# bao1029p/celestia-app

Measured on AMD Instinct MI355X. Metric: EDS+DAH squares/sec (128→256 sq, node) + RS GB/s & NMT SHA-256 hashes/sec, higher is better.
Workload: dtype u8; 1 GPU; 128x128 ODS -> 256x256 EDS + NMT row/col roots + DAH (configs[1]); k=128, global_batch=256, parallelism=squares sharded over 1 GPU(s), no collective, ods_layout=in place (Q0 of the EDS buffer)

## Files before the change

celestia-app_amd/csrc/dagpu.cpp:

```cpp
#include <hip/hip_runtime.h>
#include <stdint.h>
#include <stdio.h>
#include <stdlib.h>
#include <string.h>

#include <algorithm>
#include <cmath>
#include <map>
#include <mutex>
#include <string>
#include <vector>

#include "../../include/dagpu.h"
#include "host_sha256.hpp"
#include "kernels.hpp"
#include "runtime.hpp"

using namespace dagpu;

namespace {

size_t eds_bytes(uint64_t k) { return 4ull * k * k * kSS; }
size_t ods_bytes(uint64_t k) { return 1ull * k * k * kSS; }

int enqueue_rs(dagpu_ctx* ctx, uint32_t k, size_t n, const uint8_t* d_ods, uint8_t* d_eds,
               hipStream_t s, hipEvent_t ev_rows = nullptr) {
  const long w = 2L * k;
  const long esq = (long)eds_bytes(k);
  EncodeArgs ra{};
  if (d_ods) {
    ra.in = d_ods;
    ra.in_sq_stride = (long)ods_bytes(k);
    ra.in_vec_stride = (long)k * kSS;
    ra.in_shard_stride = kSS;
    ra.copy = d_eds;
    ra.copy_sq_stride = esq;
    ra.copy_vec_stride = w * kSS;
    ra.copy_shard_stride = kSS;
  } else {
    ra.in = d_eds;
    ra.in_sq_stride = esq;
    ra.in_vec_stride = w * kSS;
    ra.in_shard_stride = kSS;
    ra.copy = nullptr;
  }
  ra.out = d_eds + (long)k * kSS;
  ra.out_sq_stride = esq;
  ra.out_vec_stride = w * kSS;
  ra.out_shard_stride = kSS;
  ra.nsq = (long)n;
  ra.nvec = k;
  ra.nchunk = 1;
  ra.shard_bytes = kSS;
  {
    ProfScope p(ctx, 0, s);
    HIP_TRY(ctx, launch_rs_encode((int)k, ra, s));
  }
  stage_mark(ctx, DAGPU_STAGE_ROWS, s);
  if (ev_rows) HIP_TRY(ctx, hipEventRecord(ev_rows, s));
  EncodeArgs ca{};
  ca.in = d_eds;
  ca.in_sq_stride = esq;
  ca.in_vec_stride = kSS;
  ca.in_shard_stride = w * kSS;
  ca.out = d_eds + (long)k * w * kSS;
  ca.out_sq_stride = esq;
  ca.out_vec_stride = kSS;
  ca.out_shard_stride = w * kSS;
  ca.copy = nullptr;
  ca.nsq = (long)n;
  ca.nvec = w;
  ca.nchunk = 1;
  ca.shard_bytes = kSS;
  {
    ProfScope p(ctx, 1, s);
    HIP_TRY(ctx, launch_rs_encode((int)k, ca, s));
  }
  stage_mark(ctx, DAGPU_STAGE_COLS, s);
  return DAGPU_OK;
}

int enqueue_roots(dagpu_ctx* ctx, uint32_t k, size_t n, const uint8_t* d_eds, uint8_t* d_rr,
                  uint8_t* d_cr, uint8_t* d_dah, int32_t* d_status, void* d_ws, hipStream_t s) {
  SquareArgs sa{};
  sa.eds = d_eds;
  sa.eds_sq_stride = (long)eds_bytes(k);
  sa.k = (int)k;
  sa.nsq = (long)n;
  nmt_workspace_carve(sa, d_ws);
  sa.row_roots = d_rr;
  sa.col_roots = d_cr;
  sa.dah = d_dah;
  sa.status = d_status;
  sa.k = (int)k;
  sa.nsq = (long)n;
  HIP_TRY(ctx, hipMemsetAsync(d_status, 0, n * sizeof(int32_t), s));
  {
    ProfScope p(ctx, 2, s);
    HIP_TRY(ctx, launch_nmt_leaves(sa, s));
  }
  stage_mark(ctx, DAGPU_STAGE_LEAVES, s);
  {
    ProfScope p(ctx, 3, s);
    HIP_TRY(ctx, launch_nmt_trees(sa, s));
  }
  stage_mark(ctx, DAGPU_STAGE_TREES, s);
  if (d_dah) {
    ProfScope p(ctx, 4, s);
    HIP_TRY(ctx, launch_dah(sa, s));
  }
  stage_mark(ctx, DAGPU_STAGE_DAH, s);
  return DAGPU_OK;
}

size_t pipeline_chunk(uint32_t k, size_t n) {
  size_t m = (size_t(128) << 20) / ods_bytes(k);
  const long v = sw_long(SW_PIPELINE_CHUNK);
  if (v > 0) m = (size_t)v;
  return m < 1 ? 1 : (m > n ? n : m);
}

int finish_status(dagpu_ctx* ctx, const int32_t* st, size_t n, int32_t* status) {
  int first = DAGPU_OK;
  for (size_t i = 0; i < n; i++) {
    int v = (st[i] & kStatusPushOrder) ? DAGPU_ERR_PUSH_ORDER : DAGPU_OK;
    if (status) status[i] = v;
    if (v && !first) first = v;
  }
  if (first) set_err(ctx, first, "invalid push order: namespaces of original data square are not sorted");
  return first;
}

int run_group_pipelined(dagpu_ctx* ctx, uint32_t k, size_t n, size_t m, const uint8_t* ods,
                        uint8_t* eds_out, uint8_t* rr, uint8_t* cr, uint8_t* dah, int32_t* status) {
  const size_t w = 2 * (size_t)k;
  const size_t rb = w * kNodeSize, ob = ods_bytes(k), eb = eds_bytes(k);
  const size_t wsb = dagpu_workspace_size(k, m);
  hipStream_t s = ctx->stream, cs = ctx->copy_stream;
  HIP_TRY(ctx, ctx->ods.ensure(2 * m * ob));
  HIP_TRY(ctx, ctx->eds.ensure(2 * m * eb));
  HIP_TRY(ctx, ctx->rr.ensure(2 * m * rb));
  HIP_TRY(ctx, ctx->cr.ensure(2 * m * rb));
  HIP_TRY(ctx, ctx->dah.ensure(2 * m * 32));
  HIP_TRY(ctx, ctx->status.ensure(2 * m * sizeof(int32_t)));
  HIP_TRY(ctx, ctx->ws.ensure(2 * wsb));
  const size_t hslot = m * (2 * rb + 32 + sizeof(int32_t));
  HIP_TRY(ctx, ctx->h_out.ensure(2 * hslot));
  std::vector<int32_t> st(n);
  const size_t nchunks = (n + m - 1) / m;
  auto slot_dev = [&](DevBuf& b, size_t per, int slot) { return (uint8_t*)b.p + slot * m * per; };
  auto slot_host = [&](int slot) { return (uint8_t*)ctx->h_out.p + slot * hslot; };
  auto drain = [&](size_t c) -> int {
    const int slot = (int)(c & 1);
    const size_t off = c * m, cnt = (n - off < m) ? n - off : m;
    HIP_TRY(ctx, hipEventSynchronize(ctx->ev_done[slot]));
    const uint8_t* h = slot_host(slot);
    memcpy(rr + off * rb, h, cnt * rb);
    memcpy(cr + off * rb, h + m * rb, cnt * rb);
    memcpy(dah + off * 32, h + 2 * m * rb, cnt * 32);
    memcpy(st.data() + off, h + 2 * m * rb + m * 32, cnt * sizeof(int32_t));
    return DAGPU_OK;
  };
  for (size_t c = 0; c < nchunks; c++) {
    const int slot = (int)(c & 1);
    const size_t off = c * m, cnt = (n - off < m) ? n - off : m;
    if (c >= 2) {
      int rc = drain(c - 2);
      if (rc) return rc;
      HIP_TRY(ctx, hipStreamWaitEvent(cs, ctx->ev_done[slot], 0));
    }
    uint8_t* d_ods = slot_dev(ctx->ods, ob, slot);
    uint8_t* d_eds = slot_dev(ctx->eds, eb, slot);
    uint8_t* d_rr = slot_dev(ctx->rr, rb, slot);
    uint8_t* d_cr = slot_dev(ctx->cr, rb, slot);
    uint8_t* d_dah = slot_dev(ctx->dah, 32, slot);
    int32_t* d_st = (int32_t*)slot_dev(ctx->status, sizeof(int32_t), slot);
    HIP_TRY(ctx, hipMemcpyAsync(d_ods, ods + off * ob, cnt * ob, hipMemcpyHostToDevice, cs));
    HIP_TRY(ctx, hipEventRecord(ctx->ev_loaded[slot], cs));
    HIP_TRY(ctx, hipStreamWaitEvent(s, ctx->ev_loaded[slot], 0));
    int rc = enqueue_rs(ctx, k, cnt, d_ods, d_eds, s);
    if (rc) return rc;
    rc = enqueue_roots(ctx, k, cnt, d_eds, d_rr, d_cr, d_dah, d_st, (uint8_t*)ctx->ws.p + slot * wsb, s);
    if (rc) return rc;
    if (eds_out)
      HIP_TRY(ctx, hipMemcpyAsync(eds_out + off * eb, d_eds, cnt * eb, hipMemcpyDeviceToHost, s));
    uint8_t* h = slot_host(slot);
    HIP_TRY(ctx, hipMemcpyAsync(h, d_rr, cnt * rb, hipMemcpyDeviceToHost, s));
    HIP_TRY(ctx, hipMemcpyAsync(h + m * rb, d_cr, cnt * rb, hipMemcpyDeviceToHost, s));
    HIP_TRY(ctx, hipMemcpyAsync(h + 2 * m * rb, d_dah, cnt * 32, hipMemcpyDeviceToHost, s));
    HIP_TRY(ctx, hipMemcpyAsync(h + 2 * m * rb + m * 32, d_st, cnt * sizeof(int32_t), hipMemcpyDeviceToHost, s));
    HIP_TRY(ctx, hipEventRecord(ctx->ev_done[slot], s));
  }
  for (size_t c = nchunks >= 2 ? nchunks - 2 : 0; c < nchunks; c++) {
    int rc = drain(c);
// ... 275 lines not shown
                            row_roots + o_root[i], col_roots + o_root[i], dah + 32 * i, st.data());
    if (rc && rc != DAGPU_ERR_PUSH_ORDER) return rc;
    for (size_t t = i; t < j; t++) {
      if (status) status[t] = st[t - i];
      if (st[t - i] && !first) first = st[t - i];
    }
    i = j;
  }
  return first;
}

int dagpu_extend_rs_device(dagpu_ctx* ctx, uint32_t k, size_t n, const uint8_t* d_ods,
                           uint8_t* d_eds, void* stream) {
  if (!ctx || !d_eds) return DAGPU_ERR_ARG;
  int rc = check_k(ctx, k);
  if (rc) return rc;
  return enqueue_rs(ctx, k, n, d_ods, d_eds, (hipStream_t)stream);
}

int dagpu_roots_device(dagpu_ctx* ctx, uint32_t k, size_t n, const uint8_t* d_eds,
                       uint8_t* d_row_roots, uint8_t* d_col_roots, uint8_t* d_dah,
                       int32_t* d_status, void* d_workspace, void* stream) {
  if (!ctx || !d_eds || !d_row_roots || !d_col_roots || !d_dah || !d_status || !d_workspace)
    return DAGPU_ERR_ARG;
  int rc = check_k(ctx, k);
  if (rc) return rc;
  return enqueue_roots(ctx, k, n, d_eds, d_row_roots, d_col_roots, d_dah, d_status, d_workspace,
                       (hipStream_t)stream);
}

extern "C++" {
namespace dagpu {

namespace {
const char* const kSwNames[SW_COUNT] = {
    "DAGPU_PIPELINE_CHUNK", "DAGPU_PIPE_SLICES", "DAGPU_REPAIR_FILL", "DAGPU_SPLIT_SQUARE", "DAGPU_SPLIT_OVERLAP",
    "DAGPU_DAH_SPLIT",      "DAGPU_DEC_SLICED",  "DAGPU_ENC_SLICED",  "DAGPU_ENC_SLICED2",  "DAGPU_GF16_WIDE"};
thread_local const SwSnapshot* tl_sw = nullptr;
}

const char* sw(Switch s) {
  if (s < 0 || s >= SW_COUNT) return nullptr;
  if (tl_sw) return tl_sw->set[s] ? tl_sw->v[s] : nullptr;
  return getenv(kSwNames[s]);
}

long sw_long(Switch s, long dflt) {
  const char* e = sw(s);
  return e ? atol(e) : dflt;
}

void sw_snapshot(SwSnapshot* out) {
  for (int i = 0; i < SW_COUNT; i++) {
    const char* e = getenv(kSwNames[i]);
    out->set[i] = e != nullptr;
    out->v[i][0] = 0;
    if (e) snprintf(out->v[i], sizeof out->v[i], "%s", e);
  }
}

void sw_bind(const SwSnapshot* snap) { tl_sw = snap; }

hipEvent_t ev_take(dagpu_ctx* c) {
  std::lock_guard<std::mutex> g(c->ev_mu);
  if (!c->ev_pool.empty()) {
    hipEvent_t e = c->ev_pool.back();
    c->ev_pool.pop_back();
    return e;
  }
  hipEvent_t e = nullptr;
  if (hipEventCreateWithFlags(&e, hipEventDisableTiming) != hipSuccess) return nullptr;
  return e;
}

void ev_give(dagpu_ctx* c, hipEvent_t e) {
  if (!e) return;
  std::lock_guard<std::mutex> g(c->ev_mu);
  c->ev_pool.push_back(e);
}

size_t pipe_slices(dagpu_ctx* ctx, uint32_t k, size_t n) {
  const long env = sw_long(SW_PIPE_SLICES);
  if (ctx->prof) return 1;
  size_t s = env > 0 ? (size_t)env : (k >= 128 && n >= 64 ? 4 : 1);
  while (s > 1 && n / s < 8) s >>= 1;
  return s < 1 ? 1 : s;
}

hipStream_t side_stream(dagpu_ctx* ctx, hipStream_t s, int which) {
  std::lock_guard<std::mutex> g(ctx->side_mu);
  dagpu_ctx::Side* sd = nullptr;
  for (auto& p : ctx->side)
    if (p.caller == s) sd = &p;
  if (!sd) {
    if (ctx->side.size() >= dagpu_ctx::kMaxSideStreams) {
      const size_t i = (size_t)((((uint64_t)(uintptr_t)s) * 0x9E3779B97F4A7C15ull) >> 32) % ctx->side.size();
      sd = &ctx->side[i];
    } else {
      ctx->side.emplace_back();
      sd = &ctx->side.back();
      sd->caller = s;
    }
  }
  hipStream_t* slot = which == 1 ? &sd->rs_hi : &sd->rs;
  if (!*slot) {
    hipError_t e;
    if (which == 1) {
      int lo = 0, hi = 0;
      (void)hipDeviceGetStreamPriorityRange(&lo, &hi);
      e = hipStreamCreateWithPriority(slot, hipStreamNonBlocking, hi);
    } else {
      e = hipStreamCreateWithFlags(slot, hipStreamNonBlocking);
    }
    if (e != hipSuccess) {
      *slot = nullptr;
      return nullptr;
    }
  }
  return *slot;
}

}
}

int dagpu_extend_batch_device(dagpu_ctx* ctx, uint32_t k, size_t n, const uint8_t* d_ods,
                              uint8_t* d_eds, uint8_t* d_row_roots, uint8_t* d_col_roots,
                              uint8_t* d_dah, int32_t* d_status, void* d_workspace,
                              void* stream) {
  if (!ctx || !d_eds || !d_row_roots || !d_col_roots || !d_dah || !d_status || !d_workspace)
    return DAGPU_ERR_ARG;
  int rc = check_k(ctx, k);
  if (rc) return rc;
  const size_t S = pipe_slices(ctx, k, n);
  hipStream_t s = (hipStream_t)stream;
  if (S <= 1) {
    rc = enqueue_rs(ctx, k, n, d_ods, d_eds, s);
    if (rc) return rc;
    return enqueue_roots(ctx, k, n, d_eds, d_row_roots, d_col_roots, d_dah, d_status, d_workspace, s);
  }
  std::vector<hipEvent_t> ev(S + 1, nullptr);
  for (auto& e : ev)
    if (!(e = ev_take(ctx))) {
      for (auto x : ev) ev_give(ctx, x);
      return set_err(ctx, DAGPU_ERR_DEVICE, "hipEventCreate failed");
    }
  auto done = [&](int r) {
    for (auto x : ev) ev_give(ctx, x);
    return r;
  };
  hipStream_t rs = side_stream(ctx, s, 0);
  if (!rs) return done(set_err(ctx, DAGPU_ERR_DEVICE, "hipStreamCreate failed"));
  const size_t w = 2 * (size_t)k;
  if (hipEventRecord(ev[S], s) != hipSuccess || hipStreamWaitEvent(rs, ev[S], 0) != hipSuccess)
    return done(set_err(ctx, DAGPU_ERR_DEVICE, "pipeline fork failed"));
  std::vector<size_t> cut(S + 1);
  for (size_t i = 0; i <= S; i++) cut[i] = n * i / S;
  for (size_t i = 0; i < S; i++) {
    const size_t a = cut[i], b = cut[i + 1];
    rc = enqueue_rs(ctx, k, b - a, d_ods ? d_ods + a * ods_bytes(k) : nullptr, d_eds + a * eds_bytes(k), rs);
    if (rc) return done(rc);
    if (hipEventRecord(ev[i], rs) != hipSuccess) return done(set_err(ctx, DAGPU_ERR_DEVICE, "hipEventRecord failed"));
  }
  for (size_t i = 0; i < S; i++) {
    const size_t a = cut[i], b = cut[i + 1];
    if (hipStreamWaitEvent(s, ev[i], 0) != hipSuccess)
      return done(set_err(ctx, DAGPU_ERR_DEVICE, "hipStreamWaitEvent failed"));
    rc = enqueue_roots(ctx, k, b - a, d_eds + a * eds_bytes(k), d_row_roots + a * w * kNodeSize,
                       d_col_roots + a * w * kNodeSize, d_dah + a * 32, d_status + a, (uint8_t*)d_workspace, s);
    if (rc) return done(rc);
  }
  return done(DAGPU_OK);
}

int dagpu_roots(dagpu_ctx* ctx, uint32_t k, const uint8_t* eds, uint8_t* row_roots,
                uint8_t* col_roots, uint8_t* dah) {
  if (!ctx || !eds || !row_roots || !col_roots || !dah) return DAGPU_ERR_ARG;
  std::lock_guard<std::mutex> g(ctx->mu);
  (void)hipSetDevice(ctx->device);
  int rc = check_k(ctx, k);
  if (rc) return rc;
  hipStream_t s = ctx->stream;
  HostResults res;
  HIP_TRY(ctx, ctx->eds.ensure(eds_bytes(k)));
  HIP_TRY(ctx, res.alloc(ctx, k, 1));
  HIP_TRY(ctx, ctx->ws.ensure(dagpu_workspace_size(k, 1)));
  HIP_TRY(ctx, hipMemcpyAsync(ctx->eds.p, eds, eds_bytes(k), hipMemcpyHostToDevice, s));
  rc = enqueue_roots(ctx, k, 1, (const uint8_t*)ctx->eds.p, res.rr, res.cr, res.dah, res.st, ctx->ws.p, s);
  if (rc) return rc;
  HIP_TRY(ctx, res.download(ctx, s));
  HIP_TRY(ctx, hipStreamSynchronize(s));
  int32_t st = 0;
  res.deliver(ctx, row_roots, col_roots, dah, &st);
  if (st & kStatusPushOrder)
    return set_err(ctx, DAGPU_ERR_PUSH_ORDER, "invalid push order: namespaces of original data square are not sorted");
  return DAGPU_OK;
}

int dagpu_encode(dagpu_ctx* ctx, uint32_t k, size_t nvec, size_t shard_size,
                 const uint8_t* data, uint8_t* parity) {
  if (!ctx || (nvec && (!data || !parity))) return DAGPU_ERR_ARG;
  if (shard_size == 0 || shard_size % 64)
    return set_err(ctx, DAGPU_ERR_SHARE_SIZE, "shard size must be a multiple of 64");
  std::lock_guard<std::mutex> g(ctx->mu);
  (void)hipSetDevice(ctx->device);
  int rc = check_codec_k(ctx, k);
  if (rc) return rc;
  if (nvec == 0) return DAGPU_OK;
  const size_t bytes = (size_t)k * shard_size * nvec;
  hipStream_t s = ctx->stream;
  HIP_TRY(ctx, ctx->ods.ensure(bytes));
  HIP_TRY(ctx, ctx->eds.ensure(bytes));
  HIP_TRY(ctx, hipMemcpyAsync(ctx->ods.p, data, bytes, hipMemcpyHostToDevice, s));
  EncodeArgs ea{};
  ea.in = (const uint8_t*)ctx->ods.p;
  ea.out = (uint8_t*)ctx->eds.p;
  ea.copy = nullptr;
  ea.in_sq_stride = 0;
  ea.out_sq_stride = 0;
  ea.in_vec_stride = (long)k * (long)shard_size;
  ea.out_vec_stride = (long)k * (long)shard_size;
  ea.in_shard_stride = (long)shard_size;
  ea.out_shard_stride = (long)shard_size;
  ea.nsq = 1;
  ea.nvec = (long)nvec;
  ea.nchunk = (long)((shard_size + 511) / 512);
  ea.shard_bytes = (long)shard_size;
  HIP_TRY(ctx, launch_rs_encode((int)k, ea, s));
  HIP_TRY(ctx, hipMemcpyAsync(parity, ctx->eds.p, bytes, hipMemcpyDeviceToHost, s));
  HIP_TRY(ctx, hipStreamSynchronize(s));
  return DAGPU_OK;
}

int dagpu_decode(dagpu_ctx* ctx, uint32_t k, size_t nvec, size_t shard_size, uint8_t* shards,
                 const uint8_t* present) {
  if (!ctx || (nvec && (!shards || !present))) return DAGPU_ERR_ARG;
  if (shard_size == 0 || shard_size % 64)
    return set_err(ctx, DAGPU_ERR_SHARE_SIZE, "shard size must be a multiple of 64");
  std::lock_guard<std::mutex> g(ctx->mu);
  (void)hipSetDevice(ctx->device);
  int rc = check_codec_k(ctx, k);
  if (rc) return rc;
  if (nvec == 0) return DAGPU_OK;
  const size_t n = 2 * (size_t)k;
  const size_t bytes = n * shard_size * nvec;
  hipStream_t s = ctx->stream;
  HIP_TRY(ctx, ctx->eds.ensure(bytes));
  HIP_TRY(ctx, ctx->ods.ensure(n * nvec));
  const size_t errb = (size_t)rs_err_bytes((int)k) * nvec;
  HIP_TRY(ctx, ctx->ws.ensure(errb + 3 * nvec * sizeof(int32_t) + 256));
  HIP_TRY(ctx, ctx->status.ensure(sizeof(int32_t)));
  HIP_TRY(ctx, hipMemcpyAsync(ctx->eds.p, shards, bytes, hipMemcpyHostToDevice, s));
  HIP_TRY(ctx, hipMemcpyAsync(ctx->ods.p, present, n * nvec, hipMemcpyHostToDevice, s));
  HIP_TRY(ctx, hipMemsetAsync(ctx->status.p, 0, sizeof(int32_t), s));
  DecodeArgs da{};
// ... 821 lines not shown
```

celestia-app_amd/csrc/kernels.hpp:

```cpp
#pragma once
#include <hip/hip_runtime.h>
#include <stdint.h>

#include "switches.hpp"

namespace dagpu {

constexpr int kShareSize = 512;
constexpr int kNsSize = 29;
constexpr int kNodeSize = 90;
constexpr int kDigest = 32;
constexpr int kMaxK = 8192;
constexpr int kMaxCodecK = 32768;
constexpr int kMaxSplitK = 2 * kMaxK;
constexpr int kMinWideSplitParts = 8;

constexpr long rs_err_tab_off(int k) { return 4L * k; }
constexpr long rs_err_elem_bytes(int k) { return k <= 1024 ? 80 : 32; }
constexpr long rs_err_bytes(int k) { return k <= 128 ? 256 : 4L * k + 2L * k * rs_err_elem_bytes(k); }

constexpr int kStatusPushOrder = 1;

struct EncodeArgs {
  const uint8_t* in;
// ... 95 lines not shown
hipError_t launch_leo8_decode_only(const DecodeArgs& a, hipStream_t s, bool mark_present);
bool leo8_decode_sliced_applicable(const DecodeArgs& a);
hipError_t launch_leo8_decode128_sliced(const DecodeArgs& a, hipStream_t s);

hipError_t launch_leo16_encode(int k, const EncodeArgs& a, hipStream_t s);
hipError_t launch_leo16_errlocs(const DecodeArgs& a, hipStream_t s);
hipError_t launch_leo16_decode_only(const DecodeArgs& a, hipStream_t s, bool mark_present);
hipError_t launch_leo16w_encode(int k, const EncodeArgs& a, hipStream_t s);
hipError_t launch_leo16w_errlocs(const DecodeArgs& a, hipStream_t s);
hipError_t launch_leo16w_decode_only(const DecodeArgs& a, hipStream_t s, bool mark_present);
hipError_t launch_rs_prepare(int k);
hipError_t leo16w_prepare();
hipError_t launch_rs_encode(int k, const EncodeArgs& a, hipStream_t s);
hipError_t launch_rs_errlocs(const DecodeArgs& a, hipStream_t s);
hipError_t launch_errloc_heads2(const DecodeArgs& a, const DecodeArgs* a1, hipStream_t s);
hipError_t launch_rs_errlocs_only(const DecodeArgs& a, hipStream_t s);
hipError_t launch_rs_decode_only(const DecodeArgs& a, hipStream_t s, bool mark_present);
hipError_t launch_rs_decode(const DecodeArgs& a, hipStream_t s, bool mark_present);

constexpr int kRepByz = 4;
constexpr int kRepIncomplete = 8;
hipError_t launch_axis_complete(const uint8_t* present, int k, long nsq, int32_t* complete, hipStream_t s,
                                int32_t* ncomplete = nullptr);
hipError_t launch_verify_roots(const uint8_t* exp_rr, const uint8_t* exp_cr, const uint8_t* got_rr,
                               const uint8_t* got_cr, const int32_t* complete_now,
                               const int32_t* complete_before, int k, long nsq, int32_t* bits,
                               int32_t* root_bad, hipStream_t s);
struct PlanArgs {
  const int32_t* counts;
  int32_t* flags;
  int32_t* fill;
  int32_t* pair_list;
  int32_t* pair_count;
  int32_t* pair_list_rev;
  int32_t* pair_count_rev;
  int32_t* known;
  int32_t* deferred;
  const int32_t* nodefer;
  int32_t* ndeferred;
  int32_t* nplan;
  int k;
  long nsq;
  int axis;
};
hipError_t launch_repair_plan(const PlanArgs& p, hipStream_t s);
hipError_t launch_repair_defer_check(int32_t* deferred, const int32_t* known, int k, long nsq, int32_t* check,
                                     hipStream_t s, int32_t* nleft = nullptr);
hipError_t launch_vec_count(const DecodeArgs& a, hipStream_t s);
constexpr int kCtrRowsDec = 0, kCtrColsDec = 1, kCtrFillRows = 2, kCtrFillCols = 3, kCtrDeferred = 4,
              kCtrPairs = 5, kCtrPairsRev = 6, kCtrComplete = 7, kCtrDeferSquares = 8, kCtrDeferredPrev = 9,
              kCtrPlan = 10, kCtrRead = 13, kCtrTicket = 14, kCtrSlots = 64;
struct RoundCounters {
  int32_t* ctr;
  int32_t* host;
  int32_t seq;
};
hipError_t launch_vec_count_round(const DecodeArgs& a0, const DecodeArgs& a1, const RoundCounters& rc,
                                  hipStream_t s);
hipError_t launch_rs_mark_present(const DecodeArgs& a, const int32_t* flags, hipStream_t s,
                                  int32_t* known = nullptr);
hipError_t launch_rs_mark_round(const DecodeArgs& a, const int32_t* fill, int32_t* known, int32_t* zero4,
                                hipStream_t s);
hipError_t launch_finalize_repair(const int32_t* bits, const int32_t* complete_before, const int32_t* root_bad,
                                  const int32_t* parity_bad, int k, long nsq, int32_t* status, int32_t* byz,
                                  hipStream_t s, int32_t* pre_fail = nullptr);
hipError_t launch_restore_presence(uint8_t* present, const uint8_t* p0, const int32_t* pre_fail, int k, long nsq,
                                   hipStream_t s);

struct SquareArgs {
  const uint8_t* eds;
  long eds_sq_stride;
  uint8_t* digests;
  uint8_t* ns_table;
  uint8_t* rec_a;
  uint8_t* rec_b;
  uint8_t* row_roots;
  uint8_t* col_roots;
  uint8_t* dah;
  int32_t* status;
  int k;
  long nsq;
};

hipError_t launch_nmt_leaves(const SquareArgs& a, hipStream_t s);
size_t nmt_workspace_bytes(int k, long nsq);
void nmt_workspace_carve(SquareArgs& a, void* ws);
hipError_t launch_nmt_trees(const SquareArgs& a, hipStream_t s);
hipError_t launch_dah(const SquareArgs& a, hipStream_t s);

}
```

celestia-app_amd/csrc/nmt.hip:

```cpp
#include <hip/hip_runtime.h>
#include <stdint.h>
#include <stdlib.h>

#include "kernels.hpp"
#include "nmt_node.hpp"
#include "sha256.hpp"

namespace dagpu {

constexpr int kLeafWave = 256;

__global__ __launch_bounds__(kLeafWave) void nmt_leaf_kernel(SquareArgs a) {
  const int k = a.k;
  const long w = 2L * k;
  const long cells = w * w;
  const long total = cells * a.nsq;
  const long gid = (long)blockIdx.x * kLeafWave + threadIdx.x;
  if (gid >= total) return;
  const long sq = gid / cells;
  const long cell = gid - sq * cells;
  const long r = cell / w, c = cell - (cell / w) * w;
  const bool q0 = (r < k) && (c < k);
  const uint4* src = (const uint4*)(a.eds + sq * a.eds_sq_stride + cell * kShareSize);
  uint32_t st[8], ns[8];
  share_leaf_sha256(src, q0, st, ns);
  if (q0) {
    uint4* nsp = (uint4*)(a.ns_table + (sq * k * k + r * k + c) * 32);
    nsp[0] = make_uint4(ns[0], ns[1], ns[2], ns[3]);
    nsp[1] = make_uint4(ns[4], ns[5], ns[6], ns[7]);
  }
  uint4* out = (uint4*)(a.digests + gid * kDigest);
  out[0] = make_uint4(bswap32(st[0]), bswap32(st[1]), bswap32(st[2]), bswap32(st[3]));
  out[1] = make_uint4(bswap32(st[4]), bswap32(st[5]), bswap32(st[6]), bswap32(st[7]));
}

__device__ __forceinline__ void load_ns(const uint8_t* share, bool q0, uint32_t (&ns)[8]) {
  if (q0) {
    const uint4* p = (const uint4*)share;
    const uint4 v0 = p[0], v1 = p[1];
    ns[0] = v0.x; ns[1] = v0.y; ns[2] = v0.z; ns[3] = v0.w;
    ns[4] = v1.x; ns[5] = v1.y; ns[6] = v1.z; ns[7] = v1.w & 0xFFu;
  } else {
#pragma unroll
    for (int i = 0; i < 7; i++) ns[i] = 0xFFFFFFFFu;
    ns[7] = 0xFFu;
  }
}

constexpr uint32_t kParityRef = 0xFFFFFFFFu;

__device__ __forceinline__ void ns_by_ref(const uint8_t* ns_sq, uint32_t ref, uint32_t (&ns)[8]) {
  if (ref == kParityRef) {
#pragma unroll
    for (int i = 0; i < 7; i++) ns[i] = 0xFFFFFFFFu;
    ns[7] = 0xFFu;
  } else {
    const uint4* p = (const uint4*)(ns_sq + (long)ref * 32);
    const uint4 v0 = p[0], v1 = p[1];
    ns[0] = v0.x; ns[1] = v0.y; ns[2] = v0.z; ns[3] = v0.w;
    ns[4] = v1.x; ns[5] = v1.y; ns[6] = v1.z; ns[7] = v1.w;
  }
}

__device__ __forceinline__ void level_coords(long gid, int w, int per, long& sq, int& axis, int& idx, int& p) {
  const long blk = 2L * w * per;
  sq = gid / blk;
  const long g = gid - sq * blk;
  axis = g >= (long)w * per;
  const long g2 = g - (axis ? (long)w * per : 0);
  if (axis == 0) { idx = (int)(g2 / per); p = (int)(g2 - (long)idx * per); }
  else { p = (int)(g2 / w); idx = (int)(g2 - (long)p * w); }
}

__device__ __forceinline__ long level_rec(long sq, int w, int per, int axis, int idx, int p) {
  const long base = sq * 2L * w * per;
  return axis == 0 ? base + (long)idx * per + p : base + (long)w * per + (long)p * w + idx;
}

__global__ __launch_bounds__(256) void nmt_level1_kernel(SquareArgs a, uint8_t* out_rec, int final_level) {
  const int k = a.k;
  const int w = 2 * k;
  const int half = w / 2;
  const long gid = (long)blockIdx.x * 256 + threadIdx.x;
  const long total = a.nsq * 2L * w * half;
  if (gid >= total) return;
  long sq;
  int axis, idx, p;
  level_coords(gid, w, half, sq, axis, idx, p);
  const uint8_t* dig = a.digests + sq * (long)w * w * kDigest;
  const uint8_t* ns_sq = a.ns_table + sq * (long)k * k * 32;
  const int j0 = 2 * p, j1 = 2 * p + 1;
  const long cell0 = axis == 0 ? (long)idx * w + j0 : (long)j0 * w + idx;
  const long cell1 = axis == 0 ? (long)idx * w + j1 : (long)j1 * w + idx;
  const bool q00 = (idx < k) && (j0 < k), q01 = (idx < k) && (j1 < k);
  const uint32_t ref0 = q00 ? (axis == 0 ? (uint32_t)(idx * k + j0) : (uint32_t)(j0 * k + idx)) : kParityRef;
  const uint32_t ref1 = q01 ? (axis == 0 ? (uint32_t)(idx * k + j1) : (uint32_t)(j1 * k + idx)) : kParityRef;
  uint32_t nl[8], nr[8], dl[8], dr[8];
  ns_by_ref(ns_sq, ref0, nl);
  ns_by_ref(ns_sq, ref1, nr);
  load_digest(dig + cell0 * kDigest, dl);
  load_digest(dig + cell1 * kDigest, dr);
  if (q01) {
    bool bad = ns_less(nr, nl);
    if (j1 + 1 < k) {
      const uint32_t ref2 = axis == 0 ? (uint32_t)(idx * k + j1 + 1) : (uint32_t)((j1 + 1) * k + idx);
      uint32_t n2[8];
      ns_by_ref(ns_sq, ref2, n2);
      bad |= ns_less(n2, nr);
    }
    if (bad) atomicOr(&a.status[sq], kStatusPushOrder);
  }
  uint32_t st[8];
  const bool lpar = ns_is_parity(nl), rpar = ns_is_parity(nr);
  if (__all(lpar && rpar)) {
// ... 150 lines not shown
  }
#pragma unroll
  for (int j = 0; j < 8; j++) out[j] = bswap32(st[j]);
}

__global__ __launch_bounds__(kDahThreads) void dah_kernel(SquareArgs a) {
  extern __shared__ __attribute__((aligned(16))) uint32_t lds[];
  const long sq = blockIdx.x;
  const int w = 2 * a.k;
  const int n = 2 * w;
  const int C = n < kDahChunk ? n : kDahChunk;
  uint32_t* sub = lds + (C + C / 2) * 8;
  for (int c0 = 0; c0 < n; c0 += C) {
    for (int i = threadIdx.x; i < C; i += kDahThreads) dah_leaf(a, sq, c0 + i, lds + i * 8);
    __syncthreads();
    const uint32_t* r = rfc_reduce(lds, lds + C * 8, C);
    if (threadIdx.x < 8) sub[(c0 / C) * 8 + threadIdx.x] = r[threadIdx.x];
    __syncthreads();
  }
  const uint32_t* root = rfc_reduce(sub, lds, n / C);
  if (threadIdx.x < 8) {
    uint32_t* out = (uint32_t*)(a.dah + sq * 32);
    out[threadIdx.x] = root[threadIdx.x];
  }
}

constexpr int kDahSub = 64;
__global__ __launch_bounds__(kDahSub) void dah_sub_kernel(SquareArgs a) {
  __shared__ __attribute__((aligned(16))) uint32_t buf[2][kDahSub * 8];
  const int n = 4 * a.k, per = n / kDahSub;
  const long sq = blockIdx.x / per;
  const int b = (int)(blockIdx.x % per);
  const int i = threadIdx.x;
  dah_leaf(a, sq, b * kDahSub + i, buf[0] + i * 8);
  int cur = kDahSub, src = 0;
  while (cur > 1) {
    __syncthreads();
    const int next = cur / 2;
    if (i < next) {
      uint32_t m[32];
#pragma unroll
      for (int j = 0; j < 32; j++) m[j] = 0;
      uint32_t lft[8], rgt[8];
#pragma unroll
      for (int j = 0; j < 8; j++) {
        lft[j] = buf[src][(2 * i) * 8 + j];
        rgt[j] = buf[src][(2 * i + 1) * 8 + j];
      }
      m[0] = 0x01u;
      put_bytes<1>(m, lft);
      put_bytes<33>(m, rgt);
      m[65 >> 2] |= 0x80u << (8 * (65 & 3));
      uint32_t st[8];
      sha256_init(st);
#pragma unroll
      for (int blk = 0; blk < 2; blk++) {
        uint32_t wv[16];
#pragma unroll
        for (int j = 0; j < 16; j++) wv[j] = bswap32(m[16 * blk + j]);
        if (blk == 1) { wv[14] = 0; wv[15] = 65u * 8u; }
        sha256_compress(st, wv);
      }
#pragma unroll
      for (int j = 0; j < 8; j++) buf[src ^ 1][i * 8 + j] = bswap32(st[j]);
    }
    src ^= 1;
    cur = next;
  }
  __syncthreads();
  if (i < 8) ((uint32_t*)a.digests)[blockIdx.x * 8 + i] = buf[src][i];
}

__global__ __launch_bounds__(kDahThreads) void dah_top_kernel(SquareArgs a) {
  extern __shared__ __attribute__((aligned(16))) uint32_t lds[];
  const long sq = blockIdx.x;
  const int per = 4 * a.k / kDahSub;
  const uint32_t* sub = (const uint32_t*)a.digests + sq * per * 8;
  for (int i = threadIdx.x; i < per * 8; i += kDahThreads) lds[i] = sub[i];
  __syncthreads();
  const uint32_t* root = rfc_reduce(lds, lds + per * 8, per);
  if (threadIdx.x < 8) ((uint32_t*)(a.dah + sq * 32))[threadIdx.x] = root[threadIdx.x];
}

hipError_t launch_nmt_leaves(const SquareArgs& a, hipStream_t s) {
  const long w = 2L * a.k;
  const long total = w * w * a.nsq;
  const long blocks = (total + kLeafWave - 1) / kLeafWave;
  hipLaunchKernelGGL(nmt_leaf_kernel, dim3((unsigned)blocks), dim3(kLeafWave), 0, s, a);
  return hipGetLastError();
}

hipError_t launch_nmt_trees(const SquareArgs& a, hipStream_t s) {
  const int w = 2 * a.k;
  int levels = 0;
  while ((1 << levels) < w) levels++;
  uint8_t* bufs[2] = {a.rec_a, a.rec_b};
  {
    const long total = a.nsq * 2L * w * (w / 2);
    hipLaunchKernelGGL(nmt_level1_kernel, dim3((unsigned)((total + 255) / 256)), dim3(256), 0, s, a,
                       bufs[0], (int)(levels == 1));
    hipError_t e = hipGetLastError();
    if (e != hipSuccess) return e;
  }
  for (int L = 2; L <= levels; L++) {
    const long total = a.nsq * 2L * w * (w >> L);
    hipLaunchKernelGGL(nmt_level_kernel, dim3((unsigned)((total + 255) / 256)), dim3(256), 0, s, a,
                       (const uint8_t*)bufs[(L - 2) & 1], bufs[(L - 1) & 1], L, (int)(L == levels));
    hipError_t e = hipGetLastError();
    if (e != hipSuccess) return e;
  }
  return hipSuccess;
}

static size_t align256(size_t v) { return (v + 255) & ~(size_t)255; }

size_t nmt_workspace_bytes(int k, long nsq) {
  const size_t w = 2 * (size_t)k;
  const size_t dig = align256(w * w * kDigest * nsq);
  const size_t ns = align256((size_t)k * k * 32 * nsq);
  const size_t ra = align256(nsq * 2 * w * (w / 2) * 48);
  const size_t rb = align256(nsq * 2 * w * (w / 4 > 0 ? w / 4 : 1) * 48);
  return dig + ns + ra + rb;
}

void nmt_workspace_carve(SquareArgs& a, void* ws) {
  const size_t w = 2 * (size_t)a.k;
  uint8_t* p = (uint8_t*)ws;
  a.digests = p;
  p += align256(w * w * kDigest * a.nsq);
  a.ns_table = p;
  p += align256((size_t)a.k * a.k * 32 * a.nsq);
  a.rec_a = p;
  p += align256(a.nsq * 2 * w * (w / 2) * 48);
  a.rec_b = p;
}

static bool dah_split_enabled() {
  const char* e = sw(SW_DAH_SPLIT);
  return !(e && e[0] == '0');
}

hipError_t launch_dah(const SquareArgs& a, hipStream_t s) {
  const int n = 4 * a.k;
  if (a.k > kMaxSplitK) return hipErrorInvalidValue;
  if (a.digests && n >= 1024 && a.nsq < 64 && dah_split_enabled()) {
    const int per = n / kDahSub;
    hipLaunchKernelGGL(dah_sub_kernel, dim3((unsigned)(a.nsq * per)), dim3(kDahSub), 0, s, a);
    hipError_t e = hipGetLastError();
    if (e != hipSuccess) return e;
    const size_t lds = (size_t)(per + per / 2) * 8 * sizeof(uint32_t);
    hipLaunchKernelGGL(dah_top_kernel, dim3((unsigned)a.nsq), dim3(kDahThreads), lds, s, a);
    return hipGetLastError();
  }
  const int C = n < kDahChunk ? n : kDahChunk;
  const size_t lds = ((size_t)(C + C / 2) + (size_t)(n / C)) * 8 * sizeof(uint32_t);
  if (lds > 65536) {
    hipError_t e = hipFuncSetAttribute((const void*)dah_kernel,
                                       hipFuncAttributeMaxDynamicSharedMemorySize, (int)lds);
    if (e != hipSuccess) return e;
  }
  hipLaunchKernelGGL(dah_kernel, dim3((unsigned)a.nsq), dim3(kDahThreads), lds, s, a);
  return hipGetLastError();
}

}
```

Baseline: 22710 squares/s.

## Pipeline NMT leaf hashing by row halves and defer small tree levels to batched launch

Restructures the sliced extend pipeline. Hashing of the first k rows of leaves now starts as soon as the row-encode stage of a slice is signalled, and the remaining rows are hashed after the column stage. Tree levels are split at a cut level chosen from device occupancy: levels that fill the GPU run per slice, and the small upper levels run once over the whole batch using a workspace carve with per-batch namespace and record buffers. The status memset is folded into the leaf kernel, and the default slice count rises to 8 for batches of 256 or more, which adds more launches and more event synchronisation.

```diff
diff --git a/celestia-app_amd/csrc/dagpu.cpp b/celestia-app_amd/csrc/dagpu.cpp
--- a/celestia-app_amd/csrc/dagpu.cpp
+++ b/celestia-app_amd/csrc/dagpu.cpp
@@ -14,6 +14,7 @@
 #include "../../include/dagpu.h"
 #include "host_sha256.hpp"
 #include "kernels.hpp"
+#include "pipe_carve.hpp"
 #include "runtime.hpp"
 
 using namespace dagpu;
@@ -94,10 +95,9 @@
   sa.status = d_status;
   sa.k = (int)k;
   sa.nsq = (long)n;
-  HIP_TRY(ctx, hipMemsetAsync(d_status, 0, n * sizeof(int32_t), s));
   {
     ProfScope p(ctx, 2, s);
-    HIP_TRY(ctx, launch_nmt_leaves(sa, s));
+    HIP_TRY(ctx, launch_nmt_leaves(sa, s, 0, -1, true));
   }
   stage_mark(ctx, DAGPU_STAGE_LEAVES, s);
   {
@@ -110,6 +110,91 @@
     HIP_TRY(ctx, launch_dah(sa, s));
   }
   stage_mark(ctx, DAGPU_STAGE_DAH, s);
+  return DAGPU_OK;
+}
+
+struct EventSet {
+  dagpu_ctx* c;
+  std::vector<hipEvent_t> v;
+  explicit EventSet(dagpu_ctx* ctx) : c(ctx) {}
+  ~EventSet() {
+    for (auto e : v) ev_give(c, e);
+  }
+  bool take(size_t n) {
+    for (size_t i = 0; i < n; i++) {
+      hipEvent_t e = ev_take(c);
+      if (!e) return false;
+      v.push_back(e);
+    }
+    return true;
+  }
+};
+
+int extend_batch_sliced(dagpu_ctx* ctx, uint32_t k, size_t n, size_t S, const uint8_t* d_ods, uint8_t* d_eds,
+                        uint8_t* d_rr, uint8_t* d_cr, uint8_t* d_dah, int32_t* d_status, void* d_ws,
+                        hipStream_t s) {
+  const size_t w = 2 * (size_t)k;
+  std::vector<size_t> cut(S + 1);
+  for (size_t i = 0; i <= S; i++) cut[i] = n * i / S;
+  const size_t m = (n + S - 1) / S;
+  const int levels = nmt_levels((int)k);
+  PipeCarve pc{};
+  for (int cl = pipe_cut_level((int)k, m, nmt_level_fill_blocks()); cl < levels && !pc.defer; cl++)
+    pc = pipe_carve((int)k, n, m, cl, dagpu_workspace_size(k, n));
+  EventSet ev(ctx);
+  if (!ev.take(2 * S + 1)) return set_err(ctx, DAGPU_ERR_DEVICE, "hipEventCreate failed");
+  hipStream_t rs = side_stream(ctx, s, 0);
+  if (!rs) return set_err(ctx, DAGPU_ERR_DEVICE, "hipStreamCreate failed");
+  HIP_TRY(ctx, hipEventRecord(ev.v[2 * S], s));
+  HIP_TRY(ctx, hipStreamWaitEvent(rs, ev.v[2 * S], 0));
+  for (size_t i = 0; i < S; i++) {
+    const size_t a = cut[i], b = cut[i + 1];
+    int rc = enqueue_rs(ctx, k, b - a, d_ods ? d_ods + a * ods_bytes(k) : nullptr, d_eds + a * eds_bytes(k), rs,
+                        ev.v[S + i]);
+    if (rc) return rc;
+    HIP_TRY(ctx, hipEventRecord(ev.v[i], rs));
+  }
+  uint8_t* const ws = (uint8_t*)d_ws;
+  SquareArgs all{};
+  all.eds = d_eds;
+  all.eds_sq_stride = (long)eds_bytes(k);
+  all.k = (int)k;
+  all.nsq = (long)n;
+  all.digests = ws;
+  all.ns_table = pc.defer ? ws + pc.ns_all : nullptr;
+  all.row_roots = d_rr;
+  all.col_roots = d_cr;
+  all.dah = d_dah;
+  all.status = d_status;
+  for (size_t i = 0; i < S; i++) {
+    const size_t a = cut[i], b = cut[i + 1];
+    SquareArgs sa = all;
+    sa.eds = d_eds + a * eds_bytes(k);
+    sa.nsq = (long)(b - a);
+    sa.row_roots = d_rr + a * w * kNodeSize;
+    sa.col_roots = d_cr + a * w * kNodeSize;
+    sa.status = d_status + a;
+    if (pc.defer) {
+      sa.digests = ws + pc.digests;
+      sa.rec_a = ws + pc.rec_a;
+      sa.rec_b = ws + pc.rec_b;
+      sa.ns_table = ws + pc.ns_all + a * (size_t)k * k * 32;
+    } else {
+      nmt_workspace_carve(sa, ws);
+    }
+    HIP_TRY(ctx, hipStreamWaitEvent(s, ev.v[S + i], 0));
+    HIP_TRY(ctx, launch_nmt_leaves(sa, s, 0, (int)k, true));
+    HIP_TRY(ctx, hipStreamWaitEvent(s, ev.v[i], 0));
+    HIP_TRY(ctx, launch_nmt_leaves(sa, s, (int)k, (int)k, false));
+    uint8_t* const pp[2] = {sa.rec_b, sa.rec_a};
+    uint8_t* const cut_out = pc.defer ? ws + pc.rec_c + a * nmt_level_rec_bytes((int)k, pc.cut) : nullptr;
+    HIP_TRY(ctx, launch_nmt_tree_levels(sa, 1, pc.defer ? pc.cut : levels, pp, cut_out, s));
+  }
+  if (pc.defer) {
+    uint8_t* const pp[2] = {ws + pc.rec_c, ws + pc.rec_d};
+    HIP_TRY(ctx, launch_nmt_tree_levels(all, pc.cut + 1, levels, pp, nullptr, s));
+  }
+  HIP_TRY(ctx, launch_dah(all, s));
   return DAGPU_OK;
 }
 
@@ -551,7 +636,7 @@
 size_t pipe_slices(dagpu_ctx* ctx, uint32_t k, size_t n) {
   const long env = sw_long(SW_PIPE_SLICES);
   if (ctx->prof) return 1;
-  size_t s = env > 0 ? (size_t)env : (k >= 128 && n >= 64 ? 4 : 1);
+  size_t s = env > 0 ? (size_t)env : (k >= 128 && n >= 64 ? (n >= 256 ? 8 : 4) : 1);
   while (s > 1 && n / s < 8) s >>= 1;
   return s < 1 ? 1 : s;
 }
@@ -607,38 +692,7 @@
     if (rc) return rc;
     return enqueue_roots(ctx, k, n, d_eds, d_row_roots, d_col_roots, d_dah, d_status, d_workspace, s);
   }
-  std::vector<hipEvent_t> ev(S + 1, nullptr);
-  for (auto& e : ev)
-    if (!(e = ev_take(ctx))) {
-      for (auto x : ev) ev_give(ctx, x);
-      return set_err(ctx, DAGPU_ERR_DEVICE, "hipEventCreate failed");
-    }
-  auto done = [&](int r) {
-    for (auto x : ev) ev_give(ctx, x);
-    return r;
-  };
-  hipStream_t rs = side_stream(ctx, s, 0);
-  if (!rs) return done(set_err(ctx, DAGPU_ERR_DEVICE, "hipStreamCreate failed"));
-  const size_t w = 2 * (size_t)k;
-  if (hipEventRecord(ev[S], s) != hipSuccess || hipStreamWaitEvent(rs, ev[S], 0) != hipSuccess)
-    return done(set_err(ctx, DAGPU_ERR_DEVICE, "pipeline fork failed"));
-  std::vector<size_t> cut(S + 1);
-  for (size_t i = 0; i <= S; i++) cut[i] = n * i / S;
-  for (size_t i = 0; i < S; i++) {
-    const size_t a = cut[i], b = cut[i + 1];
-    rc = enqueue_rs(ctx, k, b - a, d_ods ? d_ods + a * ods_bytes(k) : nullptr, d_eds + a * eds_bytes(k), rs);
-    if (rc) return done(rc);
-    if (hipEventRecord(ev[i], rs) != hipSuccess) return done(set_err(ctx, DAGPU_ERR_DEVICE, "hipEventRecord failed"));
-  }
-  for (size_t i = 0; i < S; i++) {
-    const size_t a = cut[i], b = cut[i + 1];
-    if (hipStreamWaitEvent(s, ev[i], 0) != hipSuccess)
-      return done(set_err(ctx, DAGPU_ERR_DEVICE, "hipStreamWaitEvent failed"));
-    rc = enqueue_roots(ctx, k, b - a, d_eds + a * eds_bytes(k), d_row_roots + a * w * kNodeSize,
-                       d_col_roots + a * w * kNodeSize, d_dah + a * 32, d_status + a, (uint8_t*)d_workspace, s);
-    if (rc) return done(rc);
-  }
-  return done(DAGPU_OK);
+  return extend_batch_sliced(ctx, k, n, S, d_ods, d_eds, d_row_roots, d_col_roots, d_dah, d_status, d_workspace, s);
 }
 
 int dagpu_roots(dagpu_ctx* ctx, uint32_t k, const uint8_t* eds, uint8_t* row_roots,
diff --git a/celestia-app_amd/csrc/kernels.hpp b/celestia-app_amd/csrc/kernels.hpp
--- a/celestia-app_amd/csrc/kernels.hpp
+++ b/celestia-app_amd/csrc/kernels.hpp
@@ -201,10 +201,14 @@
   long nsq;
 };
 
-hipError_t launch_nmt_leaves(const SquareArgs& a, hipStream_t s);
+hipError_t launch_nmt_leaves(const SquareArgs& a, hipStream_t s, int row0 = 0, int nrows = -1,
+                             bool zero_status = false);
 size_t nmt_workspace_bytes(int k, long nsq);
 void nmt_workspace_carve(SquareArgs& a, void* ws);
 hipError_t launch_nmt_trees(const SquareArgs& a, hipStream_t s);
+hipError_t launch_nmt_tree_levels(const SquareArgs& a, int first, int last, uint8_t* const pp[2], uint8_t* last_out,
+                                  hipStream_t s);
+long nmt_level_fill_blocks();
 hipError_t launch_dah(const SquareArgs& a, hipStream_t s);
 
 }
diff --git a/celestia-app_amd/csrc/nmt.hip b/celestia-app_amd/csrc/nmt.hip
--- a/celestia-app_amd/csrc/nmt.hip
+++ b/celestia-app_amd/csrc/nmt.hip
@@ -4,23 +4,26 @@
 
 #include "kernels.hpp"
 #include "nmt_node.hpp"
+#include "pipe_carve.hpp"
 #include "sha256.hpp"
 
 namespace dagpu {
 
 constexpr int kLeafWave = 256;
 
-__global__ __launch_bounds__(kLeafWave) void nmt_leaf_kernel(SquareArgs a) {
+__global__ __launch_bounds__(kLeafWave) void nmt_leaf_kernel(SquareArgs a, int row0, int nrows, int zero_status) {
   const int k = a.k;
   const long w = 2L * k;
   const long cells = w * w;
-  const long total = cells * a.nsq;
+  const long span = nrows * w;
+  const long total = span * a.nsq;
   const long gid = (long)blockIdx.x * kLeafWave + threadIdx.x;
   if (gid >= total) return;
-  const long sq = gid / cells;
-  const long cell = gid - sq * cells;
+  const long sq = gid / span;
+  const long cell = row0 * w + (gid - sq * span);
   const long r = cell / w, c = cell - (cell / w) * w;
   const bool q0 = (r < k) && (c < k);
+  if (zero_status && cell == 0) a.status[sq] = 0;
   const uint4* src = (const uint4*)(a.eds + sq * a.eds_sq_stride + cell * kShareSize);
   uint32_t st[8], ns[8];
   share_leaf_sha256(src, q0, st, ns);
@@ -29,7 +32,7 @@
     nsp[0] = make_uint4(ns[0], ns[1], ns[2], ns[3]);
     nsp[1] = make_uint4(ns[4], ns[5], ns[6], ns[7]);
   }
-  uint4* out = (uint4*)(a.digests + gid * kDigest);
+  uint4* out = (uint4*)(a.digests + (sq * cells + cell) * kDigest);
   out[0] = make_uint4(bswap32(st[0]), bswap32(st[1]), bswap32(st[2]), bswap32(st[3]));
   out[1] = make_uint4(bswap32(st[4]), bswap32(st[5]), bswap32(st[6]), bswap32(st[7]));
 }
@@ -346,46 +349,61 @@
   if (threadIdx.x < 8) ((uint32_t*)(a.dah + sq * 32))[threadIdx.x] = root[threadIdx.x];
 }
 
-hipError_t launch_nmt_leaves(const SquareArgs& a, hipStream_t s) {
+hipError_t launch_nmt_leaves(const SquareArgs& a, hipStream_t s, int row0, int nrows, bool zero_status) {
   const long w = 2L * a.k;
-  const long total = w * w * a.nsq;
+  if (nrows < 0) nrows = (int)w - row0;
+  if (row0 < 0 || nrows <= 0 || row0 + nrows > w || (zero_status && (row0 != 0 || !a.status)))
+    return hipErrorInvalidValue;
+  const long total = nrows * w * a.nsq;
   const long blocks = (total + kLeafWave - 1) / kLeafWave;
-  hipLaunchKernelGGL(nmt_leaf_kernel, dim3((unsigned)blocks), dim3(kLeafWave), 0, s, a);
+  hipLaunchKernelGGL(nmt_leaf_kernel, dim3((unsigned)blocks), dim3(kLeafWave), 0, s, a, row0, nrows,
+                     (int)zero_status);
   return hipGetLastError();
 }
 
-hipError_t launch_nmt_trees(const SquareArgs& a, hipStream_t s) {
+hipError_t launch_nmt_tree_levels(const SquareArgs& a, int first, int last, uint8_t* const pp[2], uint8_t* last_out,
+                                  hipStream_t s) {
   const int w = 2 * a.k;
-  int levels = 0;
-  while ((1 << levels) < w) levels++;
-  uint8_t* bufs[2] = {a.rec_a, a.rec_b};
-  {
-    const long total = a.nsq * 2L * w * (w / 2);
-    hipLaunchKernelGGL(nmt_level1_kernel, dim3((unsigned)((total + 255) / 256)), dim3(256), 0, s, a,
-                       bufs[0], (int)(levels == 1));
+  const int levels = nmt_levels(a.k);
+  if (first < 1 || last > levels || first > last) return hipErrorInvalidValue;
+  for (int L = first; L <= last; L++) {
+    const uint8_t* in = pp[(L - first) & 1];
+    uint8_t* out = L == last && last_out ? last_out : pp[(L - first + 1) & 1];
+    const long total = a.nsq * 2L * w * (w >> L);
+    const dim3 grid((unsigned)((total + 255) / 256));
+    if (L == 1)
+      hipLaunchKernelGGL(nmt_level1_kernel, grid, dim3(256), 0, s, a, out, (int)(levels == 1));
+    else
+      hipLaunchKernelGGL(nmt_level_kernel, grid, dim3(256), 0, s, a, in, out, L, (int)(L == levels));
     hipError_t e = hipGetLastError();
     if (e != hipSuccess) return e;
   }
-  for (int L = 2; L <= levels; L++) {
-    const long total = a.nsq * 2L * w * (w >> L);
-    hipLaunchKernelGGL(nmt_level_kernel, dim3((unsigned)((total + 255) / 256)), dim3(256), 0, s, a,
-                       (const uint8_t*)bufs[(L - 2) & 1], bufs[(L - 1) & 1], L, (int)(L == levels));
-    hipError_t e = hipGetLastError();
-    if (e != hipSuccess) return e;
-  }
   return hipSuccess;
 }
 
-static size_t align256(size_t v) { return (v + 255) & ~(size_t)255; }
-
-size_t nmt_workspace_bytes(int k, long nsq) {
-  const size_t w = 2 * (size_t)k;
-  const size_t dig = align256(w * w * kDigest * nsq);
-  const size_t ns = align256((size_t)k * k * 32 * nsq);
-  const size_t ra = align256(nsq * 2 * w * (w / 2) * 48);
-  const size_t rb = align256(nsq * 2 * w * (w / 4 > 0 ? w / 4 : 1) * 48);
-  return dig + ns + ra + rb;
-}
+hipError_t launch_nmt_trees(const SquareArgs& a, hipStream_t s) {
+  uint8_t* const pp[2] = {a.rec_b, a.rec_a};
+  return launch_nmt_tree_levels(a, 1, nmt_levels(a.k), pp, nullptr, s);
+}
+
+long nmt_level_fill_blocks() {
+  static const long fill = [] {
+    int dev = 0, cus = 0, per_cu = 0;
+    if (hipGetDevice(&dev) != hipSuccess ||
+        hipDeviceGetAttribute(&cus, hipDeviceAttributeMultiprocessorCount, dev) != hipSuccess ||
+        hipOccupancyMaxActiveBlocksPerMultiprocessor(&per_cu, nmt_level_kernel, 256, 0) != hipSuccess ||
+        cus <= 0 || per_cu <= 0) {
+      (void)hipGetLastError();
+      return 0L;
+    }
+    return (long)cus * per_cu;
+  }();
+  return fill;
+}
+
+static size_t align256(size_t v) { return ws_align256(v); }
+
+size_t nmt_workspace_bytes(int k, long nsq) { return nmt_ws_bytes(k, nsq); }
 
 void nmt_workspace_carve(SquareArgs& a, void* ws) {
   const size_t w = 2 * (size_t)a.k;
diff --git a/celestia-app_amd/csrc/pipe_carve.hpp b/celestia-app_amd/csrc/pipe_carve.hpp
--- /dev/null
+++ b/celestia-app_amd/csrc/pipe_carve.hpp
@@ -0,0 +1,71 @@
+#pragma once
+#include <stddef.h>
+
+namespace dagpu {
+
+inline size_t ws_align256(size_t v) { return (v + 255) & ~(size_t)255; }
+
+inline int nmt_levels(int k) {
+  int levels = 0;
+  while ((1 << levels) < 2 * k) levels++;
+  return levels;
+}
+
+inline size_t nmt_level_rec_bytes(int k, int L) {
+  const size_t w = 2 * (size_t)k;
+  return 2 * w * (w >> L) * 48;
+}
+
+inline size_t nmt_ws_bytes(int k, long nsq) {
+  const size_t w = 2 * (size_t)k;
+  const size_t dig = ws_align256(w * w * 32 * nsq);
+  const size_t ns = ws_align256((size_t)k * k * 32 * nsq);
+  const size_t ra = ws_align256(nsq * 2 * w * (w / 2) * 48);
+  const size_t rb = ws_align256(nsq * 2 * w * (w / 4 > 0 ? w / 4 : 1) * 48);
+  return dig + ns + ra + rb;
+}
+
+inline int pipe_cut_level(int k, size_t m, long fill_blocks) {
+  const int levels = nmt_levels(k);
+  const size_t w = 2 * (size_t)k;
+  int cut = 1;
+  for (int L = 2; L <= levels; L++) {
+    const size_t blocks = (m * 2 * w * (w >> L) + 255) / 256;
+    if ((long)blocks < fill_blocks) break;
+    cut = L;
+  }
+  return cut;
+}
+
+struct PipeCarve {
+  bool defer;
+  int cut;
+  size_t digests, digests_bytes, rec_a, rec_a_bytes, rec_b, rec_b_bytes;
+  size_t ns_all, ns_all_bytes, rec_c, rec_c_bytes, rec_d, rec_d_bytes;
+  size_t end;
+};
+
+inline PipeCarve pipe_carve(int k, size_t n, size_t m, int cut, size_t limit) {
+  PipeCarve c{};
+  const int levels = nmt_levels(k);
+  const size_t w = 2 * (size_t)k;
+  c.cut = cut;
+  if (cut < 1 || cut >= levels || m == 0 || m >= n) return c;
+  size_t p = 0;
+  auto take = [&](size_t& off, size_t& bytes, size_t want) {
+    off = p;
+    bytes = want;
+    p += ws_align256(want);
+  };
+  take(c.digests, c.digests_bytes, w * w * 32 * m);
+  take(c.rec_a, c.rec_a_bytes, m * nmt_level_rec_bytes(k, 1));
+  take(c.rec_b, c.rec_b_bytes, m * nmt_level_rec_bytes(k, 2));
+  take(c.ns_all, c.ns_all_bytes, (size_t)k * k * 32 * n);
+  take(c.rec_c, c.rec_c_bytes, n * nmt_level_rec_bytes(k, cut));
+  take(c.rec_d, c.rec_d_bytes, n * nmt_level_rec_bytes(k, cut + 1));
+  c.end = p;
+  c.defer = p <= limit;
+  return c;
+}
+
+}
```

Measured after the change: 23010 squares/s (median of 6 runs). 1.01x the previous value.
